# vribeiro1/artspeech

Measured on AMD Instinct MI355X. Metric: articulator-frames/sec (fwd+bwd), higher is better.
Workload: dtype f32

## Files before the change

### artspeech_amd/_lib.py

```python
import ctypes as C
import os

import torch

_HERE = os.path.dirname(os.path.abspath(__file__))
LIB_PATH = os.path.join(_HERE, "libartspeech_hip.so")

c_f32p = C.c_void_p


class Dims(C.Structure):
    _fields_ = [("vocab", C.c_int32), ("n_art", C.c_int32), ("embed", C.c_int32), ("hidden", C.c_int32),
                ("n_samp", C.c_int32), ("simple", C.c_int32)]


class Layout(C.Structure):
    _fields_ = [("embedding", C.c_int64),
                ("w_ih", C.c_int64 * 2), ("b_ih", C.c_int64 * 2), ("w_hh", C.c_int64 * 2), ("b_hh", C.c_int64 * 2),
                ("lin_w", C.c_int64), ("lin_b", C.c_int64),
                ("ln1_g", C.c_int64), ("ln1_b", C.c_int64), ("w1", C.c_int64), ("b1", C.c_int64),
                ("ln2_g", C.c_int64), ("ln2_b", C.c_int64), ("w2", C.c_int64), ("b2", C.c_int64),
                ("ln3_g", C.c_int64), ("ln3_b", C.c_int64), ("w3", C.c_int64), ("b3", C.c_int64),
                ("total", C.c_int64)]

# ... 70 lines not shown
    "as_euclid_masked_fwd_bwd": (_I32, [_P, _P, _I64, _P, _I32, _I32, _I32, _I32, _F, _P, _P, _P, _S]),
    "as_euclid_masked_fwd_bwd_presigmoid": (_I32, [_P, _P, _I64, _P, _I32, _I32, _I32, _I32, _F, _P, _P, _P, _S]),
    "as_p2cp_fwd": (_I32, [_P, _I64, _I64, _I64, _I32, _P, _I64, _I64, _I64, _I32, _I64, _P, _S]),
    "as_p2cp_bwd": (_I32, [_P, _I64, _I64, _I64, _I32, _P, _I64, _I64, _I64, _I32, _I64, _P, _P, _I64, _I64, _I64, _P, _I64, _I64, _I64,
                           _S]),
    "as_p2cp_masked_partials": (_I32, []),
    "as_p2cp_masked_fwd_bwd": (_I32, [_P, _P, _I64, _P, _I32, _I32, _I32, _I32, _F, _P, _P, _P, _S]),
    "as_p2cp_utterance_mean": (_I32, [_P, _P, _I32, _I32, _I32, _F, _P, _S]),
    "as_pearson_fwd": (_I32, [_P, _I64, _I64, _P, _I64, _I64, _I32, _I32, _I32, _I32, _F, _P, _P, _S]),
    "as_tract_variables_fwd": (_I32, [_P, _I64, _I32, _I32, _P, _I32, _P, _P, _P, _P, _S]),
    "as_area_function_fwd": (_I32, [_P, _P, _I64, _I64, _I64, _I64, _I32, _D, _D, _P, _P, _S]),
    "as_evenly_spaced_fx": (_I32, [_P, _P, _I64, _I32, _I32, _P, _S]),
    "as_adam_step": (_I32, [_P, _P, _P, _P, _I64, _F, _F, _F, _F, _F, _I64, _F, _S]),
    "as_dropout_fwd": (_I32, [_P, _P, _I64, _F, C.c_uint64, _S]),
    "as_layernorm_fwd": (_I32, [_P, _P, _P, _P, _P, _P, _P, _I64, _I32, _I64, _S]),
    "as_fold_ln": (_I32, [_P, _P, _P, _P, _P, _P, _I32, _I32, _I32, _S]),
    "as_attn_softmax": (_I32, [_P, _I64, _I32, _I32, _I32, _I32, _F, _P, _P, _S]),
    "as_embed_posenc": (_I32, [_P, _I64, _P, _P, _P, _I64, _I32, _I32, _S]),
    "as_attn_softmax_bwd": (_I32, [_P, _P, _I64, _I32, _I32, _F, _S]),
    "as_attention_supported": (_I32, [_I32, _I32, _I32, _I32]),
    "as_attention_fwd": (_I32, [_P, _P, _P, _P, _P, _P, _P, _P, _I32, _I32, _I32, _I32, _I32, _I32, _F, _S]),
    "as_attention_fwd_causal": (_I32, [_P, _P, _P, _P, _P, _P, _P, _P, _I32, _I32, _I32, _I32, _I32, _I32, _F, _S]),
    "as_attention_bwd_ds": (_I32, [_P, _P, _P, _P, _P, _I32, _I32, _I32, _I32, _I32, _I32, _F, _S]),
    "as_attention_bwd_ds_causal": (_I32, [_P, _P, _P, _P, _P, _I32, _I32, _I32, _I32, _I32, _I32, _F, _S]),
    "as_attn_softmax_bwd_t": (_I32, [_P, _P, _P, _P, _P, _I32, _I32, _I32, _I32, _I32, _I32, _F, _S]),
    "as_group_reduce": (_I32, [_P, _P, _I32, _I32, _I64, _P, _S]),
    "as_layernorm_bwd": (_I32, [_P, _P, _P, _P, _P, _I64, _I32, _S]),
    "as_unfold_ln": (_I32, [_P, _P, _P, _P, _P, _P, _P, _P, _I32, _I32, _I32, _S]),
    "as_relu_bwd": (_I32, [_P, _P, _P, _I64, _S]),
    "as_add": (_I32, [_P, _P, _P, _I64, _S]),
    "as_row_scale": (_I32, [_P, _P, _P, _I64, _I32, _S]),
    "as_copy_f32": (_I32, [_P, _P, _I64, _S]),
    "as_set_overlap": (None, [_I32]),
    "as_set_matrix_arith": (None, [_I32]),
    "as_get_matrix_arith": (_I32, []),
    "as_conv3x3_stem": (_I32, [_P, _I64, _I64, _I64, _I64, _P, _P, _P, _P, _I32, _I32, _I32, _I32, _S]),
    "as_conv3x3_c32": (_I32, [_P, _P, _P, _P, _P, _I32, _I32, _I32, _S]),
    "as_ln_feat_gelu": (_I32, [_P, _P, _P, _P, _I64, _I32, _I32, _S]),
    "as_gelu": (_I32, [_P, _P, _I64, _S]),
    "as_lstm_bidir_fwd": (_I32, [_P, _P, _I64, _P, _P, _P, _I32, _I32, _I32, _P, _P, _S]),
    "as_lstm_bidir_bwd": (_I32, [_P, _P, _P, _P, _I32, _I32, _I32, _P, _S]),
    "as_gru_unidir_fwd": (_I32, [_P, _P, _P, _P, _I32, _I32, _I32, _P, _S]),
    "as_gru_unidir_fwd_gates": (_I32, [_P, _P, _P, _P, _I32, _I32, _I32, _P, _P, _S]),
    "as_gru_unidir_bwd": (_I32, [_P, _P, _P, _P, _P, _I32, _I32, _I32, _P, _P, _S]),
    "as_ln_feat_gelu_bwd": (_I32, [_P, _P, _P, _P, _P, _P, _I64, _I32, _I32, _S]),
    "as_conv3x3_stem_bwd": (_I32, [_P, _P, _P, _I64, _I64, _I64, _I64, _I32, _I32, _I32, _I32, _S]),
    "as_gelu_bwd": (_I32, [_P, _P, _P, _P, _I64, _I32, _S]),
    "as_conv3x3_c32_wgrad": (_I32, [_P, _P, _P, _P, _I32, _I32, _I32, _P, _I64, _S]),
    "as_conv3x3_stem_wgrad": (_I32, [_P, _I64, _I64, _I64, _I64, _P, _P, _P, _I32, _I32, _I32, _I32, _P, _I64, _S]),
    "as_ln_feat_gelu_param_grad": (_I32, [_P, _P, _P, _P, _I64, _I32, _I32, _P, _P, _P, _I64, _S]),
    "as_layernorm_param_grad": (_I32, [_P, _P, _I64, _I32, _P, _P, _P, _I64, _S]),
    "as_ctc_workspace_floats": (_I64, [_I32, _I32, _I32]),
    "as_ctc_loss": (_I32, [_P, _I64, _I64, _I32, _I32, _I32, _I32, _P, _I64, _P, _P, _I32, _I32, _I32, _P, _I64, _P, _S]),
    "as_ctc_grad": (_I32, [_P, _I64, _I64, _I32, _I32, _I32, _I32, _P, _I64, _P, _P, _I32, _I32, _P, _I64, _P, _P, _I32, _P, _I64,
                           _I64, _S]),
    "as_decode_top1": (_I32, [_P, _I64, _I64, _I32, _I32, _I32, _P, _I32, _P, _P, _P, _S]),
    "as_edit_distance": (_I32, [_P, _I32, _P, _P, _I32, _P, _I32, _P, _I32, _P, _S]),
    "as_align_workspace_bytes": (_I64, [_I32, _I32, _I32]),
    "as_align_counts": (_I32, [_P, _I32, _P, _P, _I32, _P, _I32, _P, _I32, _I32, _P, _P, _P, _I64, _S]),
    "as_confusion_counts": (_I32, [_P, _I32, _P, _I32, _P, _I32, _P, _I32, _I32, _P, _S]),
    "as_intersect_semipolar_grid":(_I32, [_P, _P, _I64, _I32, _I32, _I32, _P, _P, _P, _S]),
    "as_artspeech_wait_head_grads": (_I32, [_P, _P]),
    "as_gather_pad_rows": (_I32, [_P, _P, _P, _I32, _I32, _I64, _I32, _D, _P, _S]),
    "as_lin_debug_stamps": (None, [_P, _I64]),
    "as_gru_debug_stamps": (None, [_P]),
    "as_multi_mlp_supported": (_I32, [_I32, _I32, _I32, _I32, _I32]),
# ... 129 lines not shown
```

### artspeech_amd/csrc/artspeech.hip

```cpp
#include <stdlib.h>

#include <algorithm>
#include <mutex>
#include <vector>

#include "as_launch.h"
#include "gemm_internal.h"
#include "rowops.h"

namespace {

constexpr int D = AS_HEAD_HIDDEN;
constexpr int64_t SLAB_FLOATS = 16LL << 20;
constexpr int64_t SLAB2_FLOATS = 28LL << 20;

struct Carve {
    int64_t off = 0;
    int64_t take(int64_t n) {
        const int64_t o = off;
        off += as_round_up(n, 64);
        return o;
    }
};

struct HeadWs {
    int64_t xhat, rstd0, w1f, b1f, w2f, b2f, w3f, b3f, r1, r1hat, rstd1, r2, r2hat, rstd2;
    int64_t dpre3, dz2, dz1, dxhat, dw1f, dw2f, dw3f, slab, slab2, slab3, bits1, bits2, lpart, lpart_n, total;
    int64_t w1p, w2p, w3p, w2tp, w3tp, w1tp;
};
constexpr int OUT_BN = 128;

HeadWs head_ws(const as_dims& d, int64_t rows) {
    const int64_t A = d.n_art, H = d.hidden, O = 2 * d.n_samp;
    Carve c;
    HeadWs w;
    w.xhat = c.take(rows * H);
    w.rstd0 = c.take(rows);
    w.w1f = c.take(A * D * H);
    w.b1f = c.take(A * D);
    w.w2f = c.take(A * D * D);
    w.b2f = c.take(A * D);
    w.w3f = c.take(A * as_round_up(O, 32) * D);
    w.b3f = c.take(A * O);
    w.r1hat = c.take(rows * A * D);
    w.rstd1 = c.take(rows * A);
    w.r2hat = c.take(rows * A * D);
    w.rstd2 = c.take(rows * A);
// ... 115 lines not shown
            {ws + w.w3f, 1, D, (long)Opad * D, A, D, O, D, Opad, up(w.w3tp)},
            {ws + w.w1f, 1, H, 0, 1, H, A * D, (int)as_round_up(H, 128), A * D, up(w.w1tp)},
        };
        AS_STEP("head.planes", st, as_emit_planes(j, 6, st));
    }
    return 0;
}

struct Criterion { const float* tgt; long tgt_T; const int* lengths; int T; float scale; float* loss; float* dout; };

int head_fwd_impl(const as_dims& d, const as_layout& L, const float* P, const float* x, int64_t rows, float* out, float* ws,
                  hipStream_t st, const Criterion* crit = nullptr) {
    (void)P;
    const int A = d.n_art, H = d.hidden, O = 2 * d.n_samp;
    const HeadWs w = head_ws(d, rows);
    const int R = (int)rows;
    AS_STEP("head.norm0", st, as_normalize_fwd(x, ws + w.xhat, ws + w.rstd0, rows, H, st));
    const long AD = (long)A * D;
    const int Opad = (int)as_round_up(O, 32);
    unsigned long long* bits1 = reinterpret_cast<unsigned long long*>(ws + w.bits1);
    unsigned long long* bits2 = reinterpret_cast<unsigned long long*>(ws + w.bits2);
    as_lin l1{};
    l1.A = ws + w.xhat; l1.lda = H; l1.a_batch = 0;
    l1.B = ws + w.w1f; l1.ldb = H; l1.b_batch = (long)D * H; l1.b_kc = 1;
    l1.C = ws + w.r1hat; l1.ldc = AD; l1.c_batch = D;
    l1.bias = ws + w.b1f; l1.bias_batch = D;
    l1.M = R; l1.N = D; l1.K = H; l1.batch = A; l1.epi = 1;
    l1.rstd = ws + w.rstd1; l1.bits = bits1;
    const uint16_t* w1p = reinterpret_cast<const uint16_t*>(ws + w.w1p);
    const uint16_t* w2p = reinterpret_cast<const uint16_t*>(ws + w.w2p);
    if (H % 32 == 0) {
        l1.Bp = w1p; l1.bp_rows = D; l1.bp_batch = as_planes_batch_stride(D, H); l1.bp_plane = A * l1.bp_batch;
    }
    int took;
    bool crit_done = false;
    {
        AS_PROF("head.gemm1", st);
        took = as_lin_try(&l1, st);
        AS_REQUIRE(took >= 0, took, "head gemm1: launch failed");
    }
    if (!took) {
        AS_STEP("head.gemm1", st, gemm_nt(ws + w.xhat, H, ws + w.w1f, H, ws + w.r1, AD, ws + w.b1f, R, A * D, H, 1, st));
        AS_STEP("head.norm1", st, as_normalize_fwd(ws + w.r1, ws + w.r1hat, ws + w.rstd1, rows * A, D, st, bits1));
    }
    as_lin l2 = l1;
    l2.A = ws + w.r1hat; l2.lda = AD; l2.a_batch = D;
    l2.B = ws + w.w2f; l2.ldb = D; l2.b_batch = (long)D * D;
    l2.C = ws + w.r2hat; l2.bias = ws + w.b2f;
    l2.K = D; l2.rstd = ws + w.rstd2; l2.bits = bits2;
    l2.Bp = w2p; l2.bp_rows = D; l2.bp_batch = as_planes_batch_stride(D, D); l2.bp_plane = A * l2.bp_batch;
    {
        AS_PROF("head.gemm2", st);
        took = as_lin_try(&l2, st);
        AS_REQUIRE(took >= 0, took, "head gemm2: launch failed");
    }
    if (!took) {
        AS_STEP("head.gemm2", st, gemm_nt(ws + w.r1hat, AD, ws + w.w2f, D, ws + w.r2, AD, ws + w.b2f, R, D, D, 1, st, A, D,
                       (long)D * D, D, D));
        AS_STEP("head.norm2", st, as_normalize_fwd(ws + w.r2, ws + w.r2hat, ws + w.rstd2, rows * A, D, st, bits2));
    }
    as_lin l3{};
    l3.A = ws + w.r2hat; l3.lda = AD; l3.a_batch = D;
    l3.B = ws + w.w3f; l3.ldb = D; l3.b_batch = (long)Opad * D; l3.b_kc = 1;
    l3.C = out; l3.ldc = (long)A * O; l3.c_batch = O;
    l3.bias = ws + w.b3f; l3.bias_batch = O;
    l3.M = R; l3.N = O; l3.K = D; l3.batch = A; l3.act = 2; l3.epi = 0;
    {
        AS_PROF("head.gemm3", st);
        as_lin_out lo{};
        lo.A = ws + w.r2hat; lo.lda = AD; lo.a_batch = D;
        lo.B = ws + w.w3f; lo.ldb = D; lo.b_batch = (long)Opad * D; lo.b_rows = Opad;
        lo.bias = ws + w.b3f; lo.bias_batch = O;
        lo.out = out; lo.ldo = (long)A * O; lo.o_batch = O;
        lo.M = R; lo.N = O; lo.K = D; lo.batch = A;
        lo.Bp = reinterpret_cast<const uint16_t*>(ws + w.w3p); lo.bp_rows = (int)as_round_up(O, OUT_BN);
        lo.bp_batch = as_planes_batch_stride(lo.bp_rows, D); lo.bp_plane = A * lo.bp_batch;
        int n_part = 0;
        if (crit) {
            lo.tgt = crit->tgt; lo.tgt_T = crit->tgt_T; lo.lengths = crit->lengths; lo.T = crit->T; lo.scale = crit->scale;
            lo.dout = crit->dout; lo.partial = ws + w.lpart; lo.partial_capacity = w.lpart_n; lo.loss = crit->loss;
        }
        took = as_lin_out_try(&lo, &n_part, st);
        AS_REQUIRE(took >= 0, took, "head gemm3: launch failed");
        if (took && crit && n_part > 0) AS_TRY(as_loss_final(ws + w.lpart, n_part, crit->scale, crit->loss, st));
// ... 3 lines not shown
            AS_REQUIRE(took >= 0, took, "head gemm3: launch failed");
        }
    }
    if (!took)
        AS_STEP("head.gemm3", st, gemm_nt(ws + w.r2hat, AD, ws + w.w3f, D, out, (long)A * O, ws + w.b3f, R, O, D, 2, st, A, D,
                       (long)Opad * D, O, O));
    if (crit && !crit_done) {
        AS_STEP("loss", st, as_euclid_masked_fwd_bwd_presigmoid(out, crit->tgt, crit->tgt_T, crit->lengths, (int32_t)(rows / crit->T), crit->T, A,
                                                               d.n_samp, crit->scale, crit->loss, crit->dout, ws + w.lpart, st));
    }
    return 0;
}

int head_bwd_dx(const as_dims& d, const as_layout& L, const float* P, const float* out, const float* dout, int64_t rows,
                float* dx, const float* relu_src, float* ws, hipStream_t st, bool presig = false) {
    (void)L; (void)P;
    const int A = d.n_art, H = d.hidden, O = 2 * d.n_samp;
    const HeadWs w = head_ws(d, rows);
    const int R = (int)rows;
    const long AD = (long)A * D, AO = (long)A * O;
    const float* dpre3 = presig ? dout : ws + w.dpre3;
    if (!presig) AS_STEP("headb.sigmoid", st, as_sigmoid_bwd(out, dout, ws + w.dpre3, rows * AO, st));
    const int Opad = (int)as_round_up(O, 32);
    const unsigned long long* bits1 = reinterpret_cast<const unsigned long long*>(ws + w.bits1);
    const unsigned long long* bits2 = reinterpret_cast<const unsigned long long*>(ws + w.bits2);
    as_lin b3{};
    b3.A = dpre3; b3.lda = AO; b3.a_batch = O;
    b3.B = ws + w.w3f; b3.ldb = D; b3.b_batch = (long)Opad * D; b3.b_kc = 0;
    b3.C = ws + w.dz2; b3.ldc = AD; b3.c_batch = D;
    b3.M = R; b3.N = D; b3.K = Opad; b3.ka_valid = O; b3.batch = A; b3.epi = 2;
    b3.xhat = ws + w.r2hat; b3.ldx = AD; b3.x_batch = D; b3.rstd_in = ws + w.rstd2; b3.bits_in = bits2;
    b3.Bp = reinterpret_cast<const uint16_t*>(ws + w.w3tp); b3.bp_rows = D; b3.bp_batch = as_planes_batch_stride(D, Opad);
    b3.bp_plane = A * b3.bp_batch;
    int took;
    {
        AS_PROF("headb.dx3", st);
        took = as_lin_try(&b3, st);
        AS_REQUIRE(took >= 0, took, "head dx3: launch failed");
    }
    if (!took) {
        AS_STEP("headb.dx3", st, gemm_nn(dpre3, AO, ws + w.w3f, D, ws + w.dz2, AD, R, D, O, st, A, O, (long)Opad * D, D));
        AS_STEP("headb.norm2", st, as_normalize_bwd(ws + w.dz2, ws + w.r2hat, ws + w.rstd2, nullptr, ws + w.dz2, rows * A, D, st, bits2));
    }
    as_lin b2 = b3;
    b2.A = ws + w.dz2; b2.lda = AD; b2.a_batch = D;
    b2.B = ws + w.w2f; b2.b_batch = (long)D * D;
    b2.C = ws + w.dz1; b2.K = D; b2.ka_valid = D;
    b2.xhat = ws + w.r1hat; b2.rstd_in = ws + w.rstd1; b2.bits_in = bits1;
    b2.Bp = reinterpret_cast<const uint16_t*>(ws + w.w2tp); b2.bp_batch = as_planes_batch_stride(D, D); b2.bp_plane = A * b2.bp_batch;
    {
        AS_PROF("headb.dx2", st);
        took = as_lin_try(&b2, st);
        AS_REQUIRE(took >= 0, took, "head dx2: launch failed");
    }
    if (!took) {
        AS_STEP("headb.dx2", st, gemm_nn(ws + w.dz2, AD, ws + w.w2f, D, ws + w.dz1, AD, R, D, D, st, A, D, (long)D * D, D));
        AS_STEP("headb.norm1", st, as_normalize_bwd(ws + w.dz1, ws + w.r1hat, ws + w.rstd1, nullptr, ws + w.dz1, rows * A, D, st, bits1));
    }
    int dx1_slabs = 0;
    if (H <= 256 && H % 4 == 0) {
        as_lin l{};
        l.A = ws + w.dz1; l.lda = AD;
        l.Bp = reinterpret_cast<const uint16_t*>(ws + w.w1tp); l.bp_rows = (int)as_round_up(H, 128);
        l.bp_batch = as_planes_batch_stride(l.bp_rows, (int)AD); l.bp_plane = l.bp_batch;
        l.C = ws + w.slab; l.ldc = H;
        l.M = R; l.N = H; l.K = (int)AD; l.batch = 1;
        const int want = (int)std::max<int64_t>(1, std::min<int64_t>(8, 512 / std::max(1, as_cdiv(R, 64))));
        const int slabs = as_lin_plain_s6_slabs((int)AD, want);
        if ((int64_t)slabs * R * H <= SLAB_FLOATS) {
            AS_PROF("headb.dx1", st);
            const int took1 = as_lin_plain_s6(&l, want, (long)R * H, st, 2);
            AS_REQUIRE(took1 >= 0, took1, "head dx1: launch failed");
            if (took1) dx1_slabs = slabs;
        }
    }
    if (!dx1_slabs)
        AS_STEP("headb.dx1", st, gemm_nn(ws + w.dz1, AD, ws + w.w1f, H, ws + w.dxhat, H, R, H, (int)AD, st, 1, 0, 0, 0, ws + w.slab));
    AS_STEP("headb.norm0", st, as_normalize_bwd(dx1_slabs ? ws + w.slab : ws + w.dxhat, ws + w.xhat, ws + w.rstd0, relu_src, dx, rows, H, st, nullptr,
                                                 dx1_slabs ? dx1_slabs : 1, (long)R * H));
    return 0;
}

struct TrunkJob { const float* dz; const float* y; float* dW; float* db; int H; };
// ... 136 lines not shown
    }
    return p;
}
int record_heads_done(hipStream_t owner, hipStream_t s) {
    StreamState* p = state_for(owner);
    if (!p) return 0;
    const hipError_t e = hipEventRecord(p->heads, s);
    AS_REQUIRE(e == hipSuccess, (int)e, "as_artspeech_bwd: hipEventRecord failed: %s", hipGetErrorString(e));
    return 0;
}

int fork_after(hipStream_t from, hipStream_t to, hipEvent_t ev, hipEvent_t left) {
    hipError_t e = left ? hipEventRecord(ev, from) : hipSuccess;
    if (e == hipSuccess) e = hipStreamWaitEvent(to, ev, 0);
    if (e != hipSuccess) {
        as_set_error("stream fork failed: %s", hipGetErrorString(e));
        return (int)e;
    }
    return 0;
}

int fork_to(hipStream_t from, hipStream_t to, hipEvent_t ev) {
    hipError_t e = hipEventRecord(ev, from);
    if (e == hipSuccess) e = hipStreamWaitEvent(to, ev, 0);
    if (e != hipSuccess) {
        as_set_error("stream fork/join failed: %s", hipGetErrorString(e));
        return (int)e;
    }
    return 0;
}

}

extern "C" void as_set_overlap(int32_t on) {
    std::lock_guard<std::mutex> lock(g_state_mu);
    g_overlap = on ? 1 : 0;
}

extern "C" int as_artspeech_wait_head_grads(void* compute_stream, void* waiting_stream) {
    StreamState* p = state_for((hipStream_t)compute_stream);
    AS_REQUIRE(p, AS_ERR_UNSUPPORTED, "as_artspeech_wait_head_grads: as_artspeech_bwd has not run on that stream");
    const hipError_t e = hipStreamWaitEvent((hipStream_t)waiting_stream, p->heads, 0);
    AS_REQUIRE(e == hipSuccess, (int)e, "as_artspeech_wait_head_grads: hipStreamWaitEvent failed: %s", hipGetErrorString(e));
    return 0;
}

extern "C" int as_artspeech_layout(const as_dims* d, as_layout* out) {
    AS_TRY(check_dims(d, "as_artspeech_layout"));
    AS_REQUIRE(out, AS_ERR_BAD_ARG, "as_artspeech_layout: null out");
    const int64_t V = d->vocab, A = d->n_art, E = d->embed, H = d->hidden, N = d->n_samp;
    Carve c;
    as_layout L{};
    L.embedding = c.take(V * E);
    if (!d->simple) {
        const int64_t in[2] = {E, 2 * H};
        for (int l = 0; l < 2; ++l) {
            L.w_ih[l] = c.take(2 * 3 * H * in[l]);
            L.b_ih[l] = c.take(2 * 3 * H);
            L.w_hh[l] = c.take(2 * 3 * H * H);
            L.b_hh[l] = c.take(2 * 3 * H);
        }
        L.lin_w = c.take(H * 2 * H);
    } else {
        for (int l = 0; l < 2; ++l) L.w_ih[l] = L.b_ih[l] = L.w_hh[l] = L.b_hh[l] = -1;
        L.lin_w = c.take(H * E);
    }
// ... 248 lines not shown
```

### artspeech_amd/csrc/gemm_internal.h

```cpp
#pragma once
#include "as_common.h"
#include "gemm_plan.h"

int as_gemm_s6_launch(const as_gemm* g, const as_gemm_plan& p, hipStream_t st);
int as_wgrad_launch(const as_gemm* g, const as_gemm_plan& p, hipStream_t st);
int as_wgrad_multi(const as_wgrad_job* jobs, int n, float* slab, long slab_floats, int cu_budget, hipStream_t st, bool exact = false);

int as_matrix_arith();

struct as_planes_job {
    const float* B; long n_stride, k_stride, batch_stride;
    int batch, N, K, rows_pad, Kpad;
    uint16_t* out;
};
int as_emit_planes(const as_planes_job* jobs, int n, hipStream_t st);
static inline long as_planes_batch_stride(int rows_pad, int Kpad) { return (long)(Kpad / 16) * rows_pad * 16; }
static inline long as_planes_floats(int batch, int rows_pad, int Kpad) { return 3 * batch * as_planes_batch_stride(rows_pad, Kpad) / 2; }

void as_stop_event_set_raw(void* ev);
void* as_stop_event_take_raw();
inline void as_stop_event_set(hipEvent_t ev) { as_stop_event_set_raw((void*)ev); }
inline hipEvent_t as_stop_event_take() { return (hipEvent_t)as_stop_event_take_raw(); }

struct as_lin {
    const float* A; long lda, a_batch;
    const float* B; long ldb, b_batch; int b_kc;
    const uint16_t* Bp; long bp_plane, bp_batch; int bp_rows;
    float* C; long ldc, c_batch;
    const float* bias; long bias_batch;
    int M, N, K, ka_valid, batch, act, epi;
    float* rstd; unsigned long long* bits;
    const float* xhat; long ldx, x_batch; const float* rstd_in; const unsigned long long* bits_in;
    int tile_rows;
};
int as_lin_try(const as_lin* a, hipStream_t st);
int as_lin_plain_s6(const as_lin* a, int ksplit, long c_split, hipStream_t st, int waves_per_simd = 4);
static inline int as_lin_plain_s6_slabs(int K, int ksplit) {
    if (ksplit < 1) ksplit = 1;
    const int kchunk = (int)as_round_up(as_cdiv(K, ksplit), 32);
    return as_cdiv(K, kchunk);
}

struct as_lin_out {
    const float* A; long lda, a_batch;
    const float* B; long ldb, b_batch; int b_rows;
    const float* bias; long bias_batch;
    float* out; long ldo, o_batch;
    int M, N, K, batch;
    const float* tgt; long tgt_T; const int* lengths; int T; float scale;
    float* dout; float* partial; long partial_capacity;
    const uint16_t* Bp; long bp_plane, bp_batch; int bp_rows;
    float* loss;
};
int as_lin_out_try(const as_lin_out* a, int* n_partials, hipStream_t st);
int* as_arrival_counter(hipStream_t st);
int as_loss_final(const float* partial, int n, float scale, float* loss, hipStream_t st);

bool as_gru_bwd_tokens_fits(int32_t V, int32_t H, int32_t T);
int as_gru_bidir_bwd_tokens(const float* dy, const float* y, const float* gates, const float* w_hh, const int32_t* lengths,
                            int32_t B, int32_t T, int32_t H, float* dgh, const int64_t* tokens, int64_t tok_stride, int32_t V,
                            float* part, hipStream_t st);
int as_gru_bidir_fwd_tokens(const float* table, const int64_t* tokens, int64_t tok_stride, int32_t V, const float* w_hh,
                            const float* b_hh, const int32_t* lengths, int32_t B, int32_t T, int32_t H, float* y, float* gates,
                            hipStream_t st);
int as_count_bad_tokens(const int64_t* tokens, long tok_stride, int T, long rows, int V, int* count, hipStream_t st);
int as_sum_partials(const float* part, long n, int chunks, float* out, hipStream_t st);
```

### artspeech_amd/csrc/lin_f32.hip

```cpp
#include <cstdlib>

#include <type_traits>

#include "gemm_internal.h"
#include "split_arith.h"

namespace {

constexpr int BN = 256, BK = 16, NT = 512, NBUF = 3;
enum { EPI_PLAIN = 0, EPI_LNF = 1, EPI_LNB = 2 };

struct LinK {
    const float* A; long lda, a_batch;
    const float* B; long ldb, b_batch;
    const uint16_t* Bp; long bp_plane, bp_batch; int bp_rows;
    int kchunk; long c_split;
    float* C; long ldc, c_batch;
    const float* bias; long bias_batch;
    int M, N, K, ka_valid, batch, act;
    int n_big, big_per_batch, big_per_batch_rows, small_per_batch;
    int tile_rows;
    unsigned long long* dbg; long dbg_max;
    float eps;
    float* rstd;
// ... 355 lines not shown
                    fa[i][p] = *reinterpret_cast<const bf16x8*>(img + p * S6_PLANE + i * 32 * 64 + (((2 * s + lh_rd) ^ sw) * 16));
            const u32x4(&bs)[3] = bq[(2 * U + s) % 3];
            bf16x8 fb[3];
#pragma unroll
            for (int p = 0; p < 3; ++p) fb[p] = __builtin_bit_cast(bf16x8, bs[p]);
            constexpr int PA[6] = {0, 0, 0, 1, 1, 2}, PB[6] = {0, 1, 2, 0, 1, 0};
#pragma unroll
            for (int o = 0; o < 6; ++o)
#pragma unroll
                for (int i = 0; i < TME; ++i)
                    acc[i] = __builtin_amdgcn_mfma_f32_32x32x16_bf16(fa[i][PA[o]], fb[PB[o]], acc[i], 0, 0, 0);
            __builtin_amdgcn_sched_barrier(0);
            if (late == (s == 0)) a_store(aq[(U + 1) % 3], (kt & 1) ^ 1);
        }
        as_lds_barrier();
    };
    int kt = 0;
    for (; kt + 3 <= nk; kt += 3) {
        tile(IC<0>{}, kt);
        tile(IC<1>{}, kt + 1);
        tile(IC<2>{}, kt + 2);
    }
    {
        int ln = lane;
        asm volatile("" : "+v"(ln));
        lh_rd = ln >> 5;
        sw = ((ln & 31) >> 2) & 3;
        a_rd = sm + (ln & 31) * 64;
    }
    if (kt < nk) tile(IC<0>{}, kt);
    if (kt + 1 < nk) tile(IC<1>{}, kt + 1);
}

template <int EPI>
__global__ __launch_bounds__(NT, 4) void lin_s6_kernel(LinK g) {
    constexpr int EPIT = 32 * BN;
    static_assert(EPIT * 4 >= 2 * S6_BUF, "the epilogue's staging area holds both plane images");
    __shared__ __attribute__((aligned(16))) float smem[EPIT];
    int bz, m0, tm_eff;
    const int tile = blockIdx.x;
    if (tile < g.n_big) {
        bz = tile / g.big_per_batch;
        m0 = (tile - bz * g.big_per_batch) * 64;
        tm_eff = 2;
    } else {
        const int j = tile - g.n_big;
        bz = j / g.small_per_batch;
        m0 = g.big_per_batch_rows + (j - bz * g.small_per_batch) * 32;
        tm_eff = 1;
    }
    bz = __builtin_amdgcn_readfirstlane(bz);
    m0 = __builtin_amdgcn_readfirstlane(m0);
    const int tid = threadIdx.x, lane = tid & 63, wave = tid >> 6;
    f32x16 acc[2];
#pragma unroll
    for (int i = 0; i < 2; ++i)
#pragma unroll
        for (int r = 0; r < 16; ++r) acc[i][r] = 0.f;
    const uint16_t* bp = g.Bp + (long)bz * g.bp_batch;
    const unsigned b_lane = (unsigned)((wave * 32 + (lane & 31)) * 16 + (lane >> 5) * 8) * 2u;
    unsigned char* sm = reinterpret_cast<unsigned char*>(smem);
    const float* A = g.A + (long)bz * g.a_batch + (long)m0 * g.lda;
    const bool late = __builtin_amdgcn_readfirstlane(wave) >= 4;
    const bool stamp = g.dbg != nullptr && tid == 0 && blockIdx.x < g.dbg_max;
    unsigned long long* d = stamp ? g.dbg + 8L * blockIdx.x : nullptr;
    if (stamp) {
        d[0] = __builtin_amdgcn_s_memtime();
        d[4] = __builtin_amdgcn_s_memrealtime();
        d[5] = __builtin_amdgcn_s_getreg((4 - 1) << 11 | 0 << 6 | 4) | ((unsigned long long)__builtin_amdgcn_s_getreg((32 - 1) << 11 | 0 << 6 | 20) << 32);
    }
    if (tm_eff == 2) s6_main_loop<8, 2>(acc, sm, A, g.lda, g.M - m0, g.K, g.ka_valid, bp, b_lane, g.bp_plane, (long)g.bp_rows * 16, tid, lane, late, stamp ? d + 1 : nullptr);
    else s6_main_loop<8, 1>(acc, sm, A, g.lda, g.M - m0, g.K, g.ka_valid, bp, b_lane, g.bp_plane, (long)g.bp_rows * 16, tid, lane, late, stamp ? d + 1 : nullptr);
    if (stamp) d[2] = __builtin_amdgcn_s_memtime();
    lin_epilogue<2, EPI>(g, acc, smem, bz, m0, tm_eff, wave, lane);
    if (stamp) {
        asm volatile("s_waitcnt vmcnt(0)" ::: "memory");
        d[3] = __builtin_amdgcn_s_memtime();
        d[6] = __builtin_amdgcn_s_memrealtime();
    }
}

template <int NW, int WPS>
__global__ __launch_bounds__(NW * 64, WPS) void lin_s6_plain_kernel(LinK g) {
    __shared__ __attribute__((aligned(16))) unsigned char sm[2 * S6_BUF];
    int bz, m0, tm_eff;
    const int tile = blockIdx.x;
    if (tile < g.n_big) {
        bz = tile / g.big_per_batch;
        m0 = (tile - bz * g.big_per_batch) * 64;
        tm_eff = 2;
    } else {
        const int j = tile - g.n_big;
        bz = j / g.small_per_batch;
        m0 = g.big_per_batch_rows + (j - bz * g.small_per_batch) * 32;
        tm_eff = 1;
    }
    bz = __builtin_amdgcn_readfirstlane(bz);
    m0 = __builtin_amdgcn_readfirstlane(m0);
    const int tid = threadIdx.x, lane = tid & 63, wave = tid >> 6;
    const int l31 = lane & 31, lh = lane >> 5;
    const int ks = blockIdx.y, k0 = ks * g.kchunk;
    const int klen = min(g.kchunk, g.K - k0);
    const int kav = max(0, min(klen, g.ka_valid - k0));
    f32x16 acc[2];
#pragma unroll
    for (int i = 0; i < 2; ++i)
#pragma unroll
        for (int r = 0; r < 16; ++r) acc[i][r] = 0.f;
    const long bp_step = (long)g.bp_rows * 16;
    const uint16_t* bp = g.Bp + (long)bz * g.bp_batch + (k0 / 16) * bp_step;
    const unsigned b_lane = (unsigned)((wave * 32 + l31) * 16 + lh * 8) * 2u;
    const float* A = g.A + (long)bz * g.a_batch + (long)m0 * g.lda + k0;
    const bool late = __builtin_amdgcn_readfirstlane(wave) >= NW / 2;
    if (tm_eff == 2) s6_main_loop<NW, 2>(acc, sm, A, g.lda, g.M - m0, klen, kav, bp, b_lane, g.bp_plane, bp_step, tid, lane, late);
    else s6_main_loop<NW, 1>(acc, sm, A, g.lda, g.M - m0, klen, kav, bp, b_lane, g.bp_plane, bp_step, tid, lane, late);
    const int col = wave * 32 + l31;
    if (col >= g.N) return;
    const bool whole = gridDim.y == 1;
    const float bj = (whole && g.bias) ? g.bias[(long)bz * g.bias_batch + col] : 0.f;
    float* c0 = g.C + (long)ks * g.c_split + (long)bz * g.c_batch + col;
#pragma unroll
    for (int i = 0; i < 2; ++i)
#pragma unroll
        for (int r = 0; r < 16; ++r) {
            const int row = m0 + i * 32 + (r & 3) + 8 * (r >> 2) + 4 * lh;
            if (i < tm_eff && row < g.M) {
                float v = acc[i][r] + bj;
                if (whole && g.act == 1) v = as_relu(v);
                else if (whole && g.act == 2) v = as_sigmoid(v);
                c0[(long)row * g.ldc] = v;
            }
// ... 316 lines not shown
            if (valid) {
                const float dx = ox - tg[n], dy = oy - tg[Np + n];
                const float d = sqrtf(dx * dx + dy * dy);
                part += d;
                const float gg = g.scale / d;
                gx = dx * gg * ox * (1.f - ox);
                gy = dy * gg * oy * (1.f - oy);
            }
            dz[n] = gx;
            dz[Np + n] = gy;
        }
    }
    part = as_wave_sum_dpp(part);
    __shared__ float red[4];
    if (lane == 0) red[wave] = part;
    __syncthreads();
    float wg_sum = 0.f;
    if (tid == 0) wg_sum = (red[0] + red[1]) + (red[2] + red[3]);
    criterion_tail(g, tile, wg_sum, tid, red, 4);
}

template <typename K>
long tile_list(K& k, int x) {
    const int rest = k.M - x * 64;
    k.big_per_batch = x > 0 ? x : 1;
    k.big_per_batch_rows = x * 64;
    k.n_big = x * k.batch;
    k.small_per_batch = as_cdiv(rest, 32);
    const long total = (long)k.n_big + (long)k.small_per_batch * k.batch;
    if (k.small_per_batch == 0) k.small_per_batch = 1;
    return total;
}

template <bool B_KC, int EPI>
int launch(const LinK& k, hipStream_t st) {
    LinK kk = k;
    constexpr int slots = 512;
    const long units = (long)as_cdiv(k.M, 64) * k.batch;
    const long rounds = units / slots;
    int x = (int)(rounds * slots / k.batch);
    if (x > k.M / 64 || k.tile_rows == 64) x = k.M / 64;
    if (k.tile_rows == 32) x = 0;
    const long total = tile_list(kk, x);
    if (kk.Bp) {
        hipLaunchKernelGGL((lin_s6_kernel<EPI>), dim3((unsigned)total), dim3(NT), 0, st, kk);
        AS_LAUNCH_CHECK("as_lin_s6");
        return 0;
    }
    hipLaunchKernelGGL((lin_f32_kernel<64, B_KC, EPI>), dim3((unsigned)total), dim3(NT), 0, st, kk);
    AS_LAUNCH_CHECK("as_lin_f32");
    return 0;
}

unsigned long long* g_dbg = nullptr;
long g_dbg_max = 0;

}

extern "C" void as_lin_debug_stamps(uint64_t* buf, int64_t max_workgroups) {
    g_dbg = (unsigned long long*)buf;
    g_dbg_max = buf ? max_workgroups : 0;
}

int as_lin_try(const as_lin* a, hipStream_t st) {
    if (a->K % BK || a->K < BK || a->N > BN || a->N < 4 || a->M < 1 || a->batch < 1) return 0;
    if (!as_aligned16(a->A) || !as_aligned16(a->B) || a->lda % 4 || a->ldb % 4 || a->a_batch % 4 || a->b_batch % 4) return 0;
    if (!a->b_kc && a->N % 4) return 0;
    if (a->epi != EPI_PLAIN && (a->N != BN || !a->C)) return 0;
    if (a->epi == EPI_PLAIN && a->N <= BN / 2) return 0;
    if ((long)as_cdiv(a->M, 64) * a->batch > (1L << 30)) return 0;
    LinK k{};
    k.A = a->A; k.lda = a->lda; k.a_batch = a->a_batch;
    k.B = a->B; k.ldb = a->ldb; k.b_batch = a->b_batch;
    k.C = a->C; k.ldc = a->ldc; k.c_batch = a->c_batch;
    k.bias = a->bias; k.bias_batch = a->bias_batch;
    k.M = a->M; k.N = a->N; k.K = a->K; k.ka_valid = a->ka_valid > 0 ? a->ka_valid : a->K; k.batch = a->batch; k.act = a->act;
    k.tile_rows = a->tile_rows;
    k.eps = 1e-5f;
    k.dbg = g_dbg; k.dbg_max = g_dbg_max;
    k.rstd = a->rstd; k.bits = a->bits;
    k.xhat = a->xhat; k.ldx = a->ldx; k.x_batch = a->x_batch; k.rstd_in = a->rstd_in; k.bits_in = a->bits_in;
    if (k.ka_valid % 4) return 0;
    if (a->Bp && as_matrix_arith() == AS_ARITH_BF16X6 && a->K % S6_BK == 0 && a->bp_rows >= BN && as_aligned16(a->Bp) &&
        a->bp_plane % 8 == 0 && a->bp_batch % 8 == 0 && a->lda < (1L << 23)) {
        k.Bp = a->Bp; k.bp_plane = a->bp_plane; k.bp_batch = a->bp_batch; k.bp_rows = a->bp_rows;
    }
    if (a->epi == EPI_LNF) {
        if (!a->rstd || !a->bits || !a->b_kc) return 0;
        return launch<true, EPI_LNF>(k, st) == 0 ? 1 : -1;
    }
    if (a->epi == EPI_LNB) {
        if (!a->xhat || !a->rstd_in || !a->bits_in || a->b_kc) return 0;
        return launch<false, EPI_LNB>(k, st) == 0 ? 1 : -1;
    }
    if (a->b_kc) return launch<true, EPI_PLAIN>(k, st) == 0 ? 1 : -1;
    return launch<false, EPI_PLAIN>(k, st) == 0 ? 1 : -1;
}

int as_lin_plain_s6(const as_lin* a, int ksplit, long c_split, hipStream_t st, int waves_per_simd) {
    if (as_matrix_arith() != AS_ARITH_BF16X6 || !a->Bp) return 0;
    if (a->epi != EPI_PLAIN || a->K % S6_BK || a->K < S6_BK || a->N > BN || a->N < 1 || a->M < 1 || a->batch < 1 || !a->C) return 0;
    if (!as_aligned16(a->A) || a->lda % 4 || a->a_batch % 4 || a->lda >= (1L << 23)) return 0;
    if (!as_aligned16(a->Bp) || a->bp_plane % 8 || a->bp_batch % 8) return 0;
    const int nw = a->N <= 128 ? 4 : 8;
    if (a->bp_rows < nw * 32) return 0;
    if (ksplit < 1) ksplit = 1;
    if (ksplit > 1 && (a->bias || a->act)) return 0;
    LinK k{};
    k.A = a->A; k.lda = a->lda; k.a_batch = a->a_batch;
    k.Bp = a->Bp; k.bp_plane = a->bp_plane; k.bp_batch = a->bp_batch; k.bp_rows = a->bp_rows;
    k.C = a->C; k.ldc = a->ldc; k.c_batch = a->c_batch;
    k.bias = a->bias; k.bias_batch = a->bias_batch;
    k.M = a->M; k.N = a->N; k.K = a->K; k.ka_valid = a->ka_valid > 0 ? a->ka_valid : a->K; k.batch = a->batch; k.act = a->act;
    if (k.ka_valid % 4) return 0;
    k.kchunk = (int)as_round_up(as_cdiv(a->K, ksplit), S6_BK);
    ksplit = as_cdiv(a->K, k.kchunk);
    k.c_split = c_split;
    int tile = a->tile_rows;
    if (tile != 32 && tile != 64) tile = (long)as_cdiv(a->M, 64) * a->batch * ksplit >= 384 ? 64 : 32;
    const int x = tile == 64 ? a->M / 64 : 0;
    const long total = tile_list(k, x);
    if (total > (1L << 30) || ksplit > 65535) return 0;
    if (nw == 4 && waves_per_simd == 2) hipLaunchKernelGGL((lin_s6_plain_kernel<4, 2>), dim3((unsigned)total, ksplit), dim3(256), 0, st, k);
    else if (nw == 4) hipLaunchKernelGGL((lin_s6_plain_kernel<4, 4>), dim3((unsigned)total, ksplit), dim3(256), 0, st, k);
    else hipLaunchKernelGGL((lin_s6_plain_kernel<8, 4>), dim3((unsigned)total, ksplit), dim3(512), 0, st, k);
    AS_LAUNCH_CHECK("as_lin_plain_s6");
    return 1;
}

// ... 81 lines not shown
```

### include/artspeech_hip.h

```cpp
#ifndef ARTSPEECH_HIP_H
#define ARTSPEECH_HIP_H

#include <stdint.h>

#ifdef __cplusplus
extern "C" {
#endif

#define AS_ERR_BAD_ARG (-1)
#define AS_ERR_UNSUPPORTED (-2)
#define AS_ERR_WORKSPACE (-3)

#define AS_HEAD_HIDDEN 256

const char* as_version(void);
const char* as_arch(void);
const char* as_last_error(void);

typedef struct as_dims {
    int32_t vocab;
    int32_t n_art;
    int32_t embed;
    int32_t hidden;
    int32_t n_samp;
// ... 8 lines not shown
    int64_t ln1_g, ln1_b;
    int64_t w1, b1;
    int64_t ln2_g, ln2_b;
    int64_t w2, b2;
    int64_t ln3_g, ln3_b;
    int64_t w3, b3;
    int64_t total;
} as_layout;

int as_artspeech_layout(const as_dims* dims, as_layout* out);

int64_t as_artspeech_workspace_floats(const as_dims* dims, int32_t B, int32_t T);

typedef struct as_opts {
    float gru_dropout;
    uint64_t dropout_seed;
    int32_t dout_presigmoid;
    int32_t defer_dw2;
    void* fold_wait_event;
    const float* loss_targets; int64_t loss_tgt_T; float loss_scale; float* loss_out; float* loss_dout;
} as_opts;

int as_artspeech_fwd(const as_dims* dims, const float* params, const int64_t* tokens, int64_t tok_stride,
                     const int32_t* lengths, int32_t B, int32_t T, float* out, float* ws, int32_t train,
                     const as_opts* opts, void* stream);

int as_artspeech_bwd(const as_dims* dims, const float* params, const int64_t* tokens, int64_t tok_stride,
                     const int32_t* lengths, int32_t B, int32_t T, const float* out, const float* dout,
                     float* grads, float* ws, const as_opts* opts, void* stream);

int as_artspeech_dw2(const as_dims* dims, const float* params, int32_t B, int32_t T, float* grads, float* ws, void* stream);

void as_set_overlap(int32_t on);

int as_copy_f32(const float* src, float* dst, int64_t n, void* stream);

void as_set_matrix_arith(int32_t mode);
int32_t as_get_matrix_arith(void);

int as_artspeech_wait_head_grads(void* compute_stream, void* waiting_stream);


int as_gru_bidir_fwd(const float* gi, const int64_t* tokens, int64_t tok_stride, const float* w_hh,
                     const float* b_hh, const int32_t* lengths, int32_t B, int32_t T, int32_t H, float* y,
                     float* gates, void* stream);

int as_gru_bidir_bwd(const float* dy, const float* y, const float* gates, const float* w_hh,
                     const int32_t* lengths, int32_t B, int32_t T, int32_t H, float* dgi, float* dgh,
                     void* stream);

int as_lstm_bidir_fwd(const float* gi, const int64_t* tokens, int64_t tok_stride, const float* w_hh, const float* b_hh,
                      const int32_t* lengths, int32_t B, int32_t T, int32_t H, float* y, float* gates, void* stream);
int as_lstm_bidir_bwd(const float* dy, const float* gates, const float* w_hh, const int32_t* lengths, int32_t B, int32_t T,
                      int32_t H, float* dg, void* stream);

typedef struct as_gemm {
    const float* A; const float* B; float* C; const float* bias;
    int32_t M, N, K;
    int64_t a_i, a_k, b_j, b_k, ldc;
    int32_t batch; int64_t a_batch, b_batch, c_batch, bias_batch;
    int32_t act, accumulate;
    int32_t b_kshift, b_kT;
    float* splitk_ws; int64_t splitk_ws_floats;
    float* colsum; int64_t colsum_batch;
    const int64_t* a_off; const int64_t* b_off; const int64_t* c_off; const int64_t* bias_off;
    int32_t precision;
// ... 247 lines not shown
```

Measured before the change: 6.804 million.

## Fuse consecutive head GEMM pairs into one kernel processing row tiles in two phases

Adds a paired s6 GEMM kernel in which each workgroup computes its row tile for the first head layer (gemm1, or dx3 in backward) and then, after a block barrier, the same rows for the second layer (gemm2, or dx2). Because each tile only depends on rows it just produced itself, the intermediate stays in the workgroup's own recent writes and one kernel launch and its inter-kernel drain are removed. It is on by default, can be disabled through a new toggle, and is skipped while profiling. The cost is serialised phases inside each block, which lowers parallelism per launch, and the second phase relies on the first phase's writes being visible across waves within the block.

```diff
diff --git a/artspeech_amd/_lib.py b/artspeech_amd/_lib.py
--- a/artspeech_amd/_lib.py
+++ b/artspeech_amd/_lib.py
@@ -126,6 +126,7 @@
     "as_row_scale": (_I32, [_P, _P, _P, _I64, _I32, _S]),
     "as_copy_f32": (_I32, [_P, _P, _I64, _S]),
     "as_set_overlap": (None, [_I32]),
+    "as_set_head_pairing": (None, [_I32]),
     "as_set_matrix_arith": (None, [_I32]),
     "as_get_matrix_arith": (_I32, []),
     "as_conv3x3_stem": (_I32, [_P, _I64, _I64, _I64, _I64, _P, _P, _P, _P, _I32, _I32, _I32, _I32, _S]),
diff --git a/artspeech_amd/csrc/artspeech.hip b/artspeech_amd/csrc/artspeech.hip
--- a/artspeech_amd/csrc/artspeech.hip
+++ b/artspeech_amd/csrc/artspeech.hip
@@ -1,6 +1,7 @@
 #include <stdlib.h>
 
 #include <algorithm>
+#include <atomic>
 #include <mutex>
 #include <vector>
 
@@ -13,6 +14,9 @@
 constexpr int D = AS_HEAD_HIDDEN;
 constexpr int64_t SLAB_FLOATS = 16LL << 20;
 constexpr int64_t SLAB2_FLOATS = 28LL << 20;
+
+std::atomic<int> g_head_pairing{1};
+bool head_pairing() { return g_head_pairing.load(std::memory_order_relaxed) && !as_profile_active(); }
 
 struct Carve {
     int64_t off = 0;
@@ -194,24 +198,27 @@
     if (H % 32 == 0) {
         l1.Bp = w1p; l1.bp_rows = D; l1.bp_batch = as_planes_batch_stride(D, H); l1.bp_plane = A * l1.bp_batch;
     }
-    int took;
-    bool crit_done = false;
-    {
-        AS_PROF("head.gemm1", st);
-        took = as_lin_try(&l1, st);
-        AS_REQUIRE(took >= 0, took, "head gemm1: launch failed");
-    }
-    if (!took) {
-        AS_STEP("head.gemm1", st, gemm_nt(ws + w.xhat, H, ws + w.w1f, H, ws + w.r1, AD, ws + w.b1f, R, A * D, H, 1, st));
-        AS_STEP("head.norm1", st, as_normalize_fwd(ws + w.r1, ws + w.r1hat, ws + w.rstd1, rows * A, D, st, bits1));
-    }
     as_lin l2 = l1;
     l2.A = ws + w.r1hat; l2.lda = AD; l2.a_batch = D;
     l2.B = ws + w.w2f; l2.ldb = D; l2.b_batch = (long)D * D;
     l2.C = ws + w.r2hat; l2.bias = ws + w.b2f;
     l2.K = D; l2.rstd = ws + w.rstd2; l2.bits = bits2;
     l2.Bp = w2p; l2.bp_rows = D; l2.bp_batch = as_planes_batch_stride(D, D); l2.bp_plane = A * l2.bp_batch;
-    {
+    bool crit_done = false;
+    const int paired = head_pairing() ? as_lin_pair_try(&l1, &l2, st) : 0;
+    AS_REQUIRE(paired >= 0, paired, "head gemm1 + gemm2: launch failed");
+    int took = paired;
+    if (!took) {
+        AS_PROF("head.gemm1", st);
+        took = as_lin_try(&l1, st);
+        AS_REQUIRE(took >= 0, took, "head gemm1: launch failed");
+    }
+    if (!took) {
+        AS_STEP("head.gemm1", st, gemm_nt(ws + w.xhat, H, ws + w.w1f, H, ws + w.r1, AD, ws + w.b1f, R, A * D, H, 1, st));
+        AS_STEP("head.norm1", st, as_normalize_fwd(ws + w.r1, ws + w.r1hat, ws + w.rstd1, rows * A, D, st, bits1));
+    }
+    took = paired;
+    if (!took) {
         AS_PROF("head.gemm2", st);
         took = as_lin_try(&l2, st);
         AS_REQUIRE(took >= 0, took, "head gemm2: launch failed");
@@ -281,23 +288,26 @@
     b3.xhat = ws + w.r2hat; b3.ldx = AD; b3.x_batch = D; b3.rstd_in = ws + w.rstd2; b3.bits_in = bits2;
     b3.Bp = reinterpret_cast<const uint16_t*>(ws + w.w3tp); b3.bp_rows = D; b3.bp_batch = as_planes_batch_stride(D, Opad);
     b3.bp_plane = A * b3.bp_batch;
-    int took;
-    {
-        AS_PROF("headb.dx3", st);
-        took = as_lin_try(&b3, st);
-        AS_REQUIRE(took >= 0, took, "head dx3: launch failed");
-    }
-    if (!took) {
-        AS_STEP("headb.dx3", st, gemm_nn(dpre3, AO, ws + w.w3f, D, ws + w.dz2, AD, R, D, O, st, A, O, (long)Opad * D, D));
-        AS_STEP("headb.norm2", st, as_normalize_bwd(ws + w.dz2, ws + w.r2hat, ws + w.rstd2, nullptr, ws + w.dz2, rows * A, D, st, bits2));
-    }
     as_lin b2 = b3;
     b2.A = ws + w.dz2; b2.lda = AD; b2.a_batch = D;
     b2.B = ws + w.w2f; b2.b_batch = (long)D * D;
     b2.C = ws + w.dz1; b2.K = D; b2.ka_valid = D;
     b2.xhat = ws + w.r1hat; b2.rstd_in = ws + w.rstd1; b2.bits_in = bits1;
     b2.Bp = reinterpret_cast<const uint16_t*>(ws + w.w2tp); b2.bp_batch = as_planes_batch_stride(D, D); b2.bp_plane = A * b2.bp_batch;
-    {
+    const int paired = head_pairing() ? as_lin_pair_try(&b3, &b2, st) : 0;
+    AS_REQUIRE(paired >= 0, paired, "head dx3 + dx2: launch failed");
+    int took = paired;
+    if (!took) {
+        AS_PROF("headb.dx3", st);
+        took = as_lin_try(&b3, st);
+        AS_REQUIRE(took >= 0, took, "head dx3: launch failed");
+    }
+    if (!took) {
+        AS_STEP("headb.dx3", st, gemm_nn(dpre3, AO, ws + w.w3f, D, ws + w.dz2, AD, R, D, O, st, A, O, (long)Opad * D, D));
+        AS_STEP("headb.norm2", st, as_normalize_bwd(ws + w.dz2, ws + w.r2hat, ws + w.rstd2, nullptr, ws + w.dz2, rows * A, D, st, bits2));
+    }
+    took = paired;
+    if (!took) {
         AS_PROF("headb.dx2", st);
         took = as_lin_try(&b2, st);
         AS_REQUIRE(took >= 0, took, "head dx2: launch failed");
@@ -500,6 +510,8 @@
 
 }
 
+extern "C" void as_set_head_pairing(int32_t on) { g_head_pairing.store(on ? 1 : 0, std::memory_order_relaxed); }
+
 extern "C" void as_set_overlap(int32_t on) {
     std::lock_guard<std::mutex> lock(g_state_mu);
     g_overlap = on ? 1 : 0;
diff --git a/artspeech_amd/csrc/gemm_internal.h b/artspeech_amd/csrc/gemm_internal.h
--- a/artspeech_amd/csrc/gemm_internal.h
+++ b/artspeech_amd/csrc/gemm_internal.h
@@ -34,6 +34,7 @@
     int tile_rows;
 };
 int as_lin_try(const as_lin* a, hipStream_t st);
+int as_lin_pair_try(const as_lin* first, const as_lin* second, hipStream_t st);
 int as_lin_plain_s6(const as_lin* a, int ksplit, long c_split, hipStream_t st, int waves_per_simd = 4);
 static inline int as_lin_plain_s6_slabs(int K, int ksplit) {
     if (ksplit < 1) ksplit = 1;
diff --git a/artspeech_amd/csrc/lin_f32.hip b/artspeech_amd/csrc/lin_f32.hip
--- a/artspeech_amd/csrc/lin_f32.hip
+++ b/artspeech_amd/csrc/lin_f32.hip
@@ -411,13 +411,7 @@
     if (kt + 1 < nk) tile(IC<1>{}, kt + 1);
 }
 
-template <int EPI>
-__global__ __launch_bounds__(NT, 4) void lin_s6_kernel(LinK g) {
-    constexpr int EPIT = 32 * BN;
-    static_assert(EPIT * 4 >= 2 * S6_BUF, "the epilogue's staging area holds both plane images");
-    __shared__ __attribute__((aligned(16))) float smem[EPIT];
-    int bz, m0, tm_eff;
-    const int tile = blockIdx.x;
+__device__ __forceinline__ void lin_tile_of(const LinK& g, int tile, int& bz, int& m0, int& tm_eff) {
     if (tile < g.n_big) {
         bz = tile / g.big_per_batch;
         m0 = (tile - bz * g.big_per_batch) * 64;
@@ -430,7 +424,11 @@
     }
     bz = __builtin_amdgcn_readfirstlane(bz);
     m0 = __builtin_amdgcn_readfirstlane(m0);
-    const int tid = threadIdx.x, lane = tid & 63, wave = tid >> 6;
+}
+
+template <int EPI>
+__device__ __forceinline__ void lin_s6_tile(const LinK& g, float* smem, int bz, int m0, int tm_eff, int tid, unsigned long long* d) {
+    const int lane = tid & 63, wave = tid >> 6;
     f32x16 acc[2];
 #pragma unroll
     for (int i = 0; i < 2; ++i)
@@ -441,41 +439,59 @@
     unsigned char* sm = reinterpret_cast<unsigned char*>(smem);
     const float* A = g.A + (long)bz * g.a_batch + (long)m0 * g.lda;
     const bool late = __builtin_amdgcn_readfirstlane(wave) >= 4;
-    const bool stamp = g.dbg != nullptr && tid == 0 && blockIdx.x < g.dbg_max;
-    unsigned long long* d = stamp ? g.dbg + 8L * blockIdx.x : nullptr;
-    if (stamp) {
+    if (d) {
         d[0] = __builtin_amdgcn_s_memtime();
         d[4] = __builtin_amdgcn_s_memrealtime();
         d[5] = __builtin_amdgcn_s_getreg((4 - 1) << 11 | 0 << 6 | 4) | ((unsigned long long)__builtin_amdgcn_s_getreg((32 - 1) << 11 | 0 << 6 | 20) << 32);
     }
-    if (tm_eff == 2) s6_main_loop<8, 2>(acc, sm, A, g.lda, g.M - m0, g.K, g.ka_valid, bp, b_lane, g.bp_plane, (long)g.bp_rows * 16, tid, lane, late, stamp ? d + 1 : nullptr);
-    else s6_main_loop<8, 1>(acc, sm, A, g.lda, g.M - m0, g.K, g.ka_valid, bp, b_lane, g.bp_plane, (long)g.bp_rows * 16, tid, lane, late, stamp ? d + 1 : nullptr);
-    if (stamp) d[2] = __builtin_amdgcn_s_memtime();
+    if (tm_eff == 2) s6_main_loop<8, 2>(acc, sm, A, g.lda, g.M - m0, g.K, g.ka_valid, bp, b_lane, g.bp_plane, (long)g.bp_rows * 16, tid, lane, late, d ? d + 1 : nullptr);
+    else s6_main_loop<8, 1>(acc, sm, A, g.lda, g.M - m0, g.K, g.ka_valid, bp, b_lane, g.bp_plane, (long)g.bp_rows * 16, tid, lane, late, d ? d + 1 : nullptr);
+    if (d) d[2] = __builtin_amdgcn_s_memtime();
     lin_epilogue<2, EPI>(g, acc, smem, bz, m0, tm_eff, wave, lane);
-    if (stamp) {
+    if (d) {
         asm volatile("s_waitcnt vmcnt(0)" ::: "memory");
         d[3] = __builtin_amdgcn_s_memtime();
         d[6] = __builtin_amdgcn_s_memrealtime();
     }
+}
+
+constexpr int S6_EPIT = 32 * BN;
+static_assert(S6_EPIT * 4 >= 2 * S6_BUF, "the epilogue's staging area holds both plane images");
+
+template <int EPI>
+__global__ __launch_bounds__(NT, 4) void lin_s6_kernel(LinK g) {
+    __shared__ __attribute__((aligned(16))) float smem[S6_EPIT];
+    int bz, m0, tm_eff;
+    lin_tile_of(g, blockIdx.x, bz, m0, tm_eff);
+    const int tid = threadIdx.x;
+    const bool stamp = g.dbg != nullptr && tid == 0 && blockIdx.x < g.dbg_max;
+    lin_s6_tile<EPI>(g, smem, bz, m0, tm_eff, tid, stamp ? g.dbg + 8L * blockIdx.x : nullptr);
+}
+
+struct LinPairK { LinK first, second; };
+
+template <int EPI>
+__global__ __launch_bounds__(NT, 4) void lin_s6_pair_kernel(LinPairK p) {
+    __shared__ __attribute__((aligned(16))) float smem[S6_EPIT];
+    int bz, m0, tm_eff;
+    lin_tile_of(p.first, blockIdx.x, bz, m0, tm_eff);
+    auto phase = [&](const LinK& g) {
+        int tid = threadIdx.x;
+        asm volatile("" : "+v"(tid));
+        lin_s6_tile<EPI>(g, smem, bz, m0, tm_eff, tid, nullptr);
+    };
+    phase(p.first);
+    asm volatile("s_waitcnt vmcnt(0)" ::: "memory");
+    __threadfence_block();
+    __syncthreads();
+    phase(p.second);
 }
 
 template <int NW, int WPS>
 __global__ __launch_bounds__(NW * 64, WPS) void lin_s6_plain_kernel(LinK g) {
     __shared__ __attribute__((aligned(16))) unsigned char sm[2 * S6_BUF];
     int bz, m0, tm_eff;
-    const int tile = blockIdx.x;
-    if (tile < g.n_big) {
-        bz = tile / g.big_per_batch;
-        m0 = (tile - bz * g.big_per_batch) * 64;
-        tm_eff = 2;
-    } else {
-        const int j = tile - g.n_big;
-        bz = j / g.small_per_batch;
-        m0 = g.big_per_batch_rows + (j - bz * g.small_per_batch) * 32;
-        tm_eff = 1;
-    }
-    bz = __builtin_amdgcn_readfirstlane(bz);
-    m0 = __builtin_amdgcn_readfirstlane(m0);
+    lin_tile_of(g, blockIdx.x, bz, m0, tm_eff);
     const int tid = threadIdx.x, lane = tid & 63, wave = tid >> 6;
     const int l31 = lane & 31, lh = lane >> 5;
     const int ks = blockIdx.y, k0 = ks * g.kchunk;
@@ -858,16 +874,20 @@
     return total;
 }
 
+long head_tile_list(LinK& kk) {
+    constexpr int slots = 512;
+    const long units = (long)as_cdiv(kk.M, 64) * kk.batch;
+    const long rounds = units / slots;
+    int x = (int)(rounds * slots / kk.batch);
+    if (x > kk.M / 64 || kk.tile_rows == 64) x = kk.M / 64;
+    if (kk.tile_rows == 32) x = 0;
+    return tile_list(kk, x);
+}
+
 template <bool B_KC, int EPI>
 int launch(const LinK& k, hipStream_t st) {
     LinK kk = k;
-    constexpr int slots = 512;
-    const long units = (long)as_cdiv(k.M, 64) * k.batch;
-    const long rounds = units / slots;
-    int x = (int)(rounds * slots / k.batch);
-    if (x > k.M / 64 || k.tile_rows == 64) x = k.M / 64;
-    if (k.tile_rows == 32) x = 0;
-    const long total = tile_list(kk, x);
+    const long total = head_tile_list(kk);
     if (kk.Bp) {
         hipLaunchKernelGGL((lin_s6_kernel<EPI>), dim3((unsigned)total), dim3(NT), 0, st, kk);
         AS_LAUNCH_CHECK("as_lin_s6");
@@ -878,6 +898,13 @@
     return 0;
 }
 
+template <int EPI>
+int launch_pair(const LinPairK& p, long total, hipStream_t st) {
+    hipLaunchKernelGGL((lin_s6_pair_kernel<EPI>), dim3((unsigned)total), dim3(NT), 0, st, p);
+    AS_LAUNCH_CHECK("as_lin_s6_pair");
+    return 0;
+}
+
 unsigned long long* g_dbg = nullptr;
 long g_dbg_max = 0;
 
@@ -888,14 +915,17 @@
     g_dbg_max = buf ? max_workgroups : 0;
 }
 
-int as_lin_try(const as_lin* a, hipStream_t st) {
-    if (a->K % BK || a->K < BK || a->N > BN || a->N < 4 || a->M < 1 || a->batch < 1) return 0;
-    if (!as_aligned16(a->A) || !as_aligned16(a->B) || a->lda % 4 || a->ldb % 4 || a->a_batch % 4 || a->b_batch % 4) return 0;
-    if (!a->b_kc && a->N % 4) return 0;
-    if (a->epi != EPI_PLAIN && (a->N != BN || !a->C)) return 0;
-    if (a->epi == EPI_PLAIN && a->N <= BN / 2) return 0;
-    if ((long)as_cdiv(a->M, 64) * a->batch > (1L << 30)) return 0;
-    LinK k{};
+namespace {
+bool lin_args(const as_lin* a, LinK& k) {
+    if (a->K % BK || a->K < BK || a->N > BN || a->N < 4 || a->M < 1 || a->batch < 1) return false;
+    if (!as_aligned16(a->A) || !as_aligned16(a->B) || a->lda % 4 || a->ldb % 4 || a->a_batch % 4 || a->b_batch % 4) return false;
+    if (!a->b_kc && a->N % 4) return false;
+    if (a->epi != EPI_PLAIN && (a->N != BN || !a->C)) return false;
+    if (a->epi == EPI_PLAIN && a->N <= BN / 2) return false;
+    if (a->epi == EPI_LNF && (!a->rstd || !a->bits || !a->b_kc)) return false;
+    if (a->epi == EPI_LNB && (!a->xhat || !a->rstd_in || !a->bits_in || a->b_kc)) return false;
+    if ((long)as_cdiv(a->M, 64) * a->batch > (1L << 30)) return false;
+    k = LinK{};
     k.A = a->A; k.lda = a->lda; k.a_batch = a->a_batch;
     k.B = a->B; k.ldb = a->ldb; k.b_batch = a->b_batch;
     k.C = a->C; k.ldc = a->ldc; k.c_batch = a->c_batch;
@@ -903,24 +933,37 @@
     k.M = a->M; k.N = a->N; k.K = a->K; k.ka_valid = a->ka_valid > 0 ? a->ka_valid : a->K; k.batch = a->batch; k.act = a->act;
     k.tile_rows = a->tile_rows;
     k.eps = 1e-5f;
-    k.dbg = g_dbg; k.dbg_max = g_dbg_max;
     k.rstd = a->rstd; k.bits = a->bits;
     k.xhat = a->xhat; k.ldx = a->ldx; k.x_batch = a->x_batch; k.rstd_in = a->rstd_in; k.bits_in = a->bits_in;
-    if (k.ka_valid % 4) return 0;
+    if (k.ka_valid % 4) return false;
     if (a->Bp && as_matrix_arith() == AS_ARITH_BF16X6 && a->K % S6_BK == 0 && a->bp_rows >= BN && as_aligned16(a->Bp) &&
         a->bp_plane % 8 == 0 && a->bp_batch % 8 == 0 && a->lda < (1L << 23)) {
         k.Bp = a->Bp; k.bp_plane = a->bp_plane; k.bp_batch = a->bp_batch; k.bp_rows = a->bp_rows;
     }
-    if (a->epi == EPI_LNF) {
-        if (!a->rstd || !a->bits || !a->b_kc) return 0;
-        return launch<true, EPI_LNF>(k, st) == 0 ? 1 : -1;
-    }
-    if (a->epi == EPI_LNB) {
-        if (!a->xhat || !a->rstd_in || !a->bits_in || a->b_kc) return 0;
-        return launch<false, EPI_LNB>(k, st) == 0 ? 1 : -1;
-    }
+    return true;
+}
+}
+
+int as_lin_try(const as_lin* a, hipStream_t st) {
+    LinK k;
+    if (!lin_args(a, k)) return 0;
+    k.dbg = g_dbg; k.dbg_max = g_dbg_max;
+    if (a->epi == EPI_LNF) return launch<true, EPI_LNF>(k, st) == 0 ? 1 : -1;
+    if (a->epi == EPI_LNB) return launch<false, EPI_LNB>(k, st) == 0 ? 1 : -1;
     if (a->b_kc) return launch<true, EPI_PLAIN>(k, st) == 0 ? 1 : -1;
     return launch<false, EPI_PLAIN>(k, st) == 0 ? 1 : -1;
+}
+
+int as_lin_pair_try(const as_lin* first, const as_lin* second, hipStream_t st) {
+    if (first->epi != second->epi || (first->epi != EPI_LNF && first->epi != EPI_LNB)) return 0;
+    if (first->M != second->M || first->batch != second->batch || first->tile_rows != second->tile_rows) return 0;
+    if (second->A != first->C || second->lda != first->ldc || second->a_batch != first->c_batch) return 0;
+    LinPairK p;
+    if (!lin_args(first, p.first) || !lin_args(second, p.second) || !p.first.Bp || !p.second.Bp) return 0;
+    const long total = head_tile_list(p.first);
+    head_tile_list(p.second);
+    if (first->epi == EPI_LNF) return launch_pair<EPI_LNF>(p, total, st) == 0 ? 1 : -1;
+    return launch_pair<EPI_LNB>(p, total, st) == 0 ? 1 : -1;
 }
 
 int as_lin_plain_s6(const as_lin* a, int ksplit, long c_split, hipStream_t st, int waves_per_simd) {
diff --git a/include/artspeech_hip.h b/include/artspeech_hip.h
--- a/include/artspeech_hip.h
+++ b/include/artspeech_hip.h
@@ -64,6 +64,8 @@
 int as_artspeech_dw2(const as_dims* dims, const float* params, int32_t B, int32_t T, float* grads, float* ws, void* stream);
 
 void as_set_overlap(int32_t on);
+
+void as_set_head_pairing(int32_t on);
 
 int as_copy_f32(const float* src, float* dst, int64_t n, void* stream);
 
```

After: 6.839 million (median of 6 runs). About the same (+0.5%).
